# apache/paimon

Hardware: NVIDIA H100
Metric: merged rows/sec at 16 runs x 40M rows (higher is better)
Workload: dtype int64

## Files before the change

paimon_b200/csrc/device_utils.cuh:

```cuda
#pragma once

#include "pg_internal.h"

namespace pg {

__device__ __forceinline__ int warp_scan_incl(int v) {
    int lane = threadIdx.x & 31;
#pragma unroll
    for (int d = 1; d < 32; d <<= 1) {
        int n = __shfl_up_sync(0xffffffffu, v, d);
        if (lane >= d) v += n;
    }
    return v;
}

__device__ __forceinline__ int block_scan_excl(int v, int *ws, int *total) {
    int lane = threadIdx.x & 31, w = threadIdx.x >> 5, nw = blockDim.x >> 5;
    int incl = warp_scan_incl(v);
    if (lane == 31) ws[w] = incl;
    __syncthreads();
    if (w == 0) {
        int x = lane < nw ? ws[lane] : 0;
        int xi = warp_scan_incl(x);
        ws[lane] = xi - x;
// ... 120 lines not shown
    }
    if (fn == 4) {
        r = -(__int128)a;
    } else if (fn == 2) {
        r = dec_div_half_up((__int128)a * (__int128)b, dec_pow10(scale));
    } else {
        if (b == 0) {
            atomicCAS(err, KERR_NONE, a == 0 ? KERR_DEC_DIV_UNDEFINED : KERR_DEC_DIV_ZERO);
            return DecimalResult{0, false};
        }
        const uint64_t mb = b < 0 ? 0ull - ub : ub;
        uint64_t x = a < 0 ? 0ull - ua : ua, y = mb;
        while (x != 0) { const uint64_t t = y % x; y = x; x = t; }
        uint64_t den = mb / y;
        while (den % 2 == 0) den /= 2;
        while (den % 5 == 0) den /= 5;
        if (den != 1) {
            atomicCAS(err, KERR_NONE, KERR_DEC_NON_TERMINATING);
            return DecimalResult{0, false};
        }
        const __int128 n = (__int128)a * (__int128)dec_pow10(scale);
        r = dec_div_half_up(b < 0 ? -n : n, (unsigned __int128)mb);
    }
    const bool fits = dec_fits(r, precision);
    return DecimalResult{fits ? (uint64_t)(int64_t)r : 0, fits};
}

__device__ __forceinline__ uint64_t negate_fixed(int type, int width, uint64_t a) {
    if (type == PG_DOUBLE) return a ^ 0x8000000000000000ull;
    if (type == PG_FLOAT) return (uint32_t)a ^ 0x80000000u;
    return 0ull - (uint64_t)sext(a, width);
}

__device__ __forceinline__ int compare_fixed(int type, int width, uint64_t a, uint64_t b) {
    if (type == PG_DOUBLE)
        return java_double_compare(__longlong_as_double((long long)a), __longlong_as_double((long long)b));
    if (type == PG_FLOAT) return java_float_compare(__int_as_float((int)a), __int_as_float((int)b));
    int64_t x = sext(a, width), y = sext(b, width);
    return x < y ? -1 : x > y ? 1 : 0;
}

__device__ __forceinline__ int bytes_compare(const uint8_t *a, int la, const uint8_t *b, int lb) {
    int n = min(la, lb);
    for (int i = 0; i < n; i++) {
        int d = (int)a[i] - (int)b[i];
        if (d) return d;
    }
    return la - lb;
}


__device__ __forceinline__ uint32_t smem_u32(const void *p) { return (uint32_t)__cvta_generic_to_shared(p); }

__device__ __forceinline__ void mbar_init(uint64_t *bar, int count) {
    asm volatile("mbarrier.init.shared::cta.b64 [%0], %1;" ::"r"(smem_u32(bar)), "r"(count) : "memory");
}
__device__ __forceinline__ void mbar_fence_init() {
    asm volatile("fence.mbarrier_init.release.cluster;" ::: "memory");
    asm volatile("fence.proxy.async.shared::cta;" ::: "memory");
}
__device__ __forceinline__ void mbar_arrive_expect_tx(uint64_t *bar, uint32_t bytes) {
    asm volatile("mbarrier.arrive.expect_tx.shared::cta.b64 _, [%0], %1;" ::"r"(smem_u32(bar)), "r"(bytes)
                 : "memory");
}
__device__ __forceinline__ void mbar_wait(uint64_t *bar, uint32_t parity) {
    uint32_t ok;
    do {
        asm volatile(
            "{\n\t.reg .pred p;\n\t"
            "mbarrier.try_wait.parity.shared::cta.b64 p, [%1], %2;\n\t"
            "selp.u32 %0, 1, 0, p;\n\t}"
            : "=r"(ok)
            : "r"(smem_u32(bar)), "r"(parity)
            : "memory");
    } while (!ok);
}
__device__ __forceinline__ void bulk_g2s(void *dst_smem, const void *src_gmem, uint32_t bytes, uint64_t *bar) {
    asm volatile("cp.async.bulk.shared::cluster.global.mbarrier::complete_tx::bytes [%0], [%1], %2, [%3];" ::"r"(
                     smem_u32(dst_smem)),
                 "l"(src_gmem), "r"(bytes), "r"(smem_u32(bar))
                 : "memory");
}

}
```

paimon_b200/csrc/emit.cu:

```cuda
#include <stdio.h>

#include "device_utils.cuh"

namespace pg {

constexpr int kStages = 2;
constexpr int kEmitThreads = 512;
constexpr int kEmitWarps = kEmitThreads / 32;
#define kFlagAgg (1ull << 62)
#define kFlagPrefix (2ull << 62)
#define kValMask ((1ull << 62) - 1)

constexpr uint32_t kPmPosMask = 0x1FFF;
constexpr int kPmOpShift = 13;
constexpr uint32_t kPmHead = 0x8000;

struct EmitLayout {
    int rt;
    size_t stage_bytes;
    size_t total;
};
__host__ __device__ inline EmitLayout emit_layout(int k) {
    EmitLayout L;
    L.rt = kTileMax + 64 * k;
    L.stage_bytes = (((size_t)L.rt * 8 + (size_t)L.rt / 32 * 4) + 127) & ~(size_t)127;
    L.total = kStages * L.stage_bytes + (size_t)kTileMax * (2 + 2 + 1) + (PG_MAX_RUNS + 1) * 4 * 3 +
              PG_MAX_RUNS * 8 + kStages * PG_MAX_RUNS * 8 + kStages * 8 + 34 * 4 + 64;
    return L;
}

__device__ __forceinline__ bool staged_valid(const uint32_t *vw, int p) { return (vw[p >> 5] >> (p & 31)) & 1; }

template <int W> __device__ __forceinline__ uint64_t lds_fixed(const unsigned char *vals, int p);
template <> __device__ __forceinline__ uint64_t lds_fixed<1>(const unsigned char *v, int p) { return v[p]; }
template <> __device__ __forceinline__ uint64_t lds_fixed<2>(const unsigned char *v, int p) { return ((const uint16_t *)v)[p]; }
template <> __device__ __forceinline__ uint64_t lds_fixed<4>(const unsigned char *v, int p) { return ((const uint32_t *)v)[p]; }
template <> __device__ __forceinline__ uint64_t lds_fixed<8>(const unsigned char *v, int p) { return ((const uint64_t *)v)[p]; }
template <typename T> __device__ __forceinline__ T *as_global(T *p) { __builtin_assume(__isGlobal(p)); return p; }
template <int W> __device__ __forceinline__ void stg_fixed(void *d, int64_t row, uint64_t v);
template <> __device__ __forceinline__ void stg_fixed<1>(void *d, int64_t r, uint64_t v) { as_global((uint8_t *)d)[r] = (uint8_t)v; }
template <> __device__ __forceinline__ void stg_fixed<2>(void *d, int64_t r, uint64_t v) { as_global((uint16_t *)d)[r] = (uint16_t)v; }
template <> __device__ __forceinline__ void stg_fixed<4>(void *d, int64_t r, uint64_t v) { as_global((uint32_t *)d)[r] = (uint32_t)v; }
template <> __device__ __forceinline__ void stg_fixed<8>(void *d, int64_t r, uint64_t v) { as_global((uint64_t *)d)[r] = v; }

template <bool GAGG>
__device__ __forceinline__ int select_pos(const uint16_t *pm, const uint32_t *vw, int last) {
    int j = last;
    while (true) {
        uint32_t e = pm[j];
        uint32_t op = (e >> kPmOpShift) & 3;
        if (GAGG && op == OP_RETRACT) op = (e & kPmHead) ? OP_SET : OP_NOOP;
        if (op != OP_NOOP) {
            int pj = e & kPmPosMask;
            if (staged_valid(vw, pj)) return pj;
            if (op == OP_SET) return -1;
        }
        if (e & kPmHead) return -1;
        --j;
    }
}
template <bool GAGG>
__device__ __forceinline__ int select_member_idx(const uint16_t *pm, const uint32_t *vw, int last) {
    int j = last;
    while (true) {
        uint32_t e = pm[j];
        uint32_t op = (e >> kPmOpShift) & 3;
        if (GAGG && op == OP_RETRACT) op = (e & kPmHead) ? OP_SET : OP_NOOP;
        if (op != OP_NOOP) {
            if (staged_valid(vw, e & kPmPosMask)) return j;
            if (op == OP_SET) return -1;
        }
        if (e & kPmHead) return -1;
        --j;
    }
}

__device__ __forceinline__ int select_marked_idx(const uint16_t *pm, const uint32_t *gplan, uint32_t bit, int last) {
    int j = last;
    while (true) {
        if (gplan[j] & bit) return j;
        if (pm[j] & kPmHead) return -1;
        --j;
    }
}

__device__ __forceinline__ int group_first(const uint16_t *pm, int last) {
    int j = last;
    while (!(pm[j] & kPmHead)) --j;
    return j;
}

__device__ int fold_member_idx(const ColDesc &cd, const uint16_t *pm, const uint8_t *mrun, const uint32_t *vw,
                               const int32_t *offs, const uint8_t *const *cdata, int last, int32_t *err) {
    int acc = -1;
    bool initialized = false;
    for (int j = group_first(pm, last); j <= last; j++) {
        uint32_t e = pm[j];
        int op = (e >> kPmOpShift) & 3;
        if (op == OP_NOOP) continue;
        bool v = staged_valid(vw, e & kPmPosMask);
        int in = v ? j : -1;
        if (op == OP_SET) { acc = in; continue; }
        if (op == OP_RETRACT) {
            if (cd.retract == RT_IGNORE) continue;
            switch (cd.agg) {
                case PG_AGG_LAST_VALUE: acc = -1; break;
                case PG_AGG_LAST_NON_NULL_VALUE: if (v) acc = -1; break;
                case PG_AGG_PRIMARY_KEY: acc = in; break;
                default: atomicCAS(err, KERR_NONE, KERR_AGG_RETRACT); break;
            }
// ... 213 lines not shown
        if (active) {
            uint64_t val = 0;
            const int last = tv.glast[ob];
            if (cd.mode == CM_SELECT) {
                int pj = select_pos<GAGG>(tv.pm, vw, last);
                if (pj >= 0) { val = lds_fixed<W>(vals, pj); is_valid = true; }
            } else if (cd.mode == CM_GVAL || cd.mode == CM_GSEQ) {
                const uint32_t gbit = 1u << (cd.agg + (cd.mode == CM_GSEQ ? 16 : 0));
                const int j = select_marked_idx(tv.pm, ea.gplan + tv.in_base, gbit, last);
                if (j >= 0) {
                    const int pj = tv.pm[j] & kPmPosMask;
                    if (staged_valid(vw, pj)) { val = lds_fixed<W>(vals, pj); is_valid = true; }
                }
            } else if (GAGG && cd.mode == CM_GAGG) {
                fold_group_agg<false>(cd, tv.pm, ea.gagg + tv.in_base, vw, vals, last, &val, &is_valid, ea.err);
                if (!is_valid) val = 0;
            } else if (cd.mode == CM_KEY) {
                val = lds_fixed<W>(vals, tv.pm[last] & kPmPosMask); is_valid = true;
            } else if (cd.mode == CM_SEQ) {
                val = (uint64_t)ea.tmp_seq[result_index(tv, ob)]; is_valid = true;
            } else if (cd.mode == CM_KIND) {
                val = (uint8_t)ea.tmp_kind[result_index(tv, ob)]; is_valid = true;
            } else {
                fold_fixed<false>(cd, tv.pm, vw, vals, last, &val, &is_valid, ea.err);
                if (!is_valid) val = 0;
            }
            stg_fixed<W>(oc.data, tv.out_base + ob, val);
        }
        if (oc.validity != nullptr) put_validity_word(oc.validity, tv.out_base, wb, tv.n_out, is_valid);
    }
}

template <bool GAGG>
__device__ __forceinline__ void emit_decimal_column(const ColDesc &cd, const pg_out_column &oc, const TileView &tv,
                                                    const unsigned char *vals, const uint32_t *vw, const uint32_t *gagg,
                                                    int32_t *err) {
    const int tid = threadIdx.x, lane = tid & 31;
    for (int wb = (tid & ~31) - tv.o_shift; wb < tv.n_out; wb += kEmitThreads) {
        const int ob = wb + lane;
        bool is_valid = false;
        if (ob >= 0 && ob < tv.n_out) {
            uint64_t val = 0;
            const int last = tv.glast[ob];
            if (GAGG && cd.mode == CM_GAGG) fold_group_agg<true>(cd, tv.pm, gagg, vw, vals, last, &val, &is_valid, err);
            else fold_fixed<true>(cd, tv.pm, vw, vals, last, &val, &is_valid, err);
            stg_fixed<8>(oc.data, tv.out_base + ob, is_valid ? val : 0);
        }
        if (oc.validity != nullptr) put_validity_word(oc.validity, tv.out_base, wb, tv.n_out, is_valid);
    }
}

#ifdef PG_EMIT_TIMING
__device__ long long g_emit_ts[64 * 256];
#define TS(slot) do { if (tid == 0 && ts_on) g_emit_ts[(ts_tile) * 256 + (slot)] = clock64(); } while (0)
#else
#define TS(slot) do { } while (0)
#endif

struct PassEnt { ColDesc cd; pg_out_column oc; int32_t c, pad; };
constexpr int kPassCache = 64;

template <bool GAGG>
__global__ void __launch_bounds__(kEmitThreads, 2)
k_emit(EmitArgs ea) {
    extern __shared__ __align__(128) unsigned char smem[];
    __shared__ PassEnt s_pass[kPassCache];
    const int k = ea.k, tid = threadIdx.x, lane = tid & 31, warp = tid >> 5;
    const EmitLayout L = emit_layout(k);
    auto stage_vals = [&](int s) -> unsigned char * { return smem + (size_t)s * L.stage_bytes; };
    auto stage_vw = [&](int s) -> uint32_t * { return (uint32_t *)(smem + (size_t)s * L.stage_bytes + (size_t)L.rt * 8); };
    unsigned char *p = smem + kStages * L.stage_bytes;
    uint16_t *pm = (uint16_t *)p;              p += kTileMax * 2;
    uint16_t *glast = (uint16_t *)p;           p += kTileMax * 2;
    uint8_t *mrun = (uint8_t *)p;              p += kTileMax;
    int64_t *rstart = (int64_t *)p;            p += PG_MAX_RUNS * 8;
    const uint8_t **cdata = (const uint8_t **)p; p += kStages * PG_MAX_RUNS * 8;
    uint64_t *mbar = (uint64_t *)p;            p += kStages * 8;
    int64_t *s_i64 = (int64_t *)p;             p += 16;
    int *seg = (int *)p;                       p += (PG_MAX_RUNS + 1) * 4;
    int *seg_a = (int *)p;                     p += (PG_MAX_RUNS + 1) * 4;
    int *rr = (int *)p;                        p += (PG_MAX_RUNS + 1) * 4;
    int *ws = (int *)p;                        p += 34 * 4;
    int *s_i32 = (int *)p;                     p += 16;

    if (tid == 0) {
        s_i32[0] = atomicAdd(ea.tile_counter, 1);
        for (int s = 0; s < kStages; s++) mbar_init(&mbar[s], 1);
        mbar_fence_init();
    }
    __syncthreads();
    const int tile = s_i32[0];
    if (tid < ea.n_passes && tid < kPassCache) {
        const int c = ea.col_order[tid];
        s_pass[tid].c = c;
        s_pass[tid].cd = ea.cols[c];
        s_pass[tid].oc = ea.out_cols[c];
    }
#ifdef PG_EMIT_TIMING
    const bool ts_on = tile >= 2000 && tile < 2064;
    const int ts_tile = tile - 2000;
#endif
    TS(0);
    const int plan_a = 2 * tile, plan_end = min(plan_a + 2, ea.n_plan_tiles);
    if (warp == 0) {
        int64_t b0 = 0, bm = 0, b1 = 0;
        if (lane < k) {
            b0 = ea.bounds[(int64_t)plan_a * k + lane];
            bm = ea.bounds[(int64_t)(plan_a + 1) * k + lane];
            b1 = ea.bounds[(int64_t)plan_end * k + lane];
        }
        const int len = (int)(b1 - b0), len_a = (int)(bm - b0);
        const int rlen = lane < k ? (((int)(b0 & 31) + len + 1) + 31) & ~31 : 0;
        const int i_len = warp_scan_incl(len), i_a = warp_scan_incl(len_a), i_r = warp_scan_incl(rlen);
        if (lane < k) {
            rstart[lane] = b0;
            seg[lane] = i_len - len;
            seg_a[lane] = i_a - len_a;
            rr[lane] = i_r - rlen;
        }
        if (lane == 31) { seg[k] = i_len; seg_a[k] = i_a; rr[k] = i_r; }
    }
    __syncthreads();
    const int n = seg[k];
    const int n_vw = rr[k] >> 5;
    int64_t in_base = 0;
    for (int r = 0; r < k; r++) in_base += rstart[r];

    constexpr int VT = kTileMax / kEmitThreads;
    const int p0 = tid * VT, p1 = min(p0 + VT, n);
    int my = 0;
    uint32_t emit_bits = 0;
    uint16_t *spos = glast;
    uint8_t *srun = stage_vals(1);
    const int n_a = seg_a[k];
    for (int r = 0; r < k; r++) {
        const int len_a = seg_a[r + 1] - seg_a[r], len = seg[r + 1] - seg[r];
        const int p0r = rr[r] + (int)(rstart[r] & 31);
        const int sb0 = n_a + (seg[r] - seg_a[r]);
        for (int j = tid; j < len; j += kEmitThreads) {
            const int idx = j < len_a ? seg_a[r] + j : sb0 + (j - len_a);
            spos[idx] = (uint16_t)(p0r + j);
            srun[idx] = (uint8_t)r;
        }
    }
    __syncthreads();
    for (int i = p0; i < p1; i++) {
        uint16_t e = ea.plan[in_base + i];
        int slot = (e & kPlanSlotMask) + (i < n_a ? 0 : n_a);
        mrun[i] = srun[slot];
        uint32_t pos = spos[slot];
        uint32_t op = (e >> kPlanOpShift) & 3;
        pm[i] = (uint16_t)(pos | (op << kPmOpShift) | ((e & kPlanHead) ? kPmHead : 0));
        if ((e & kPlanHead) && (e & kPlanEmit)) { my++; emit_bits |= 1u << (i - p0); }
    }
    int n_out = 0;
    int o = block_scan_excl(my, ws, &n_out);
    for (int i = p0; i < p1; i++) {
        if (emit_bits & (1u << (i - p0))) {
            int e = i + 1;
            while (e < n && !(pm[e] & kPmHead)) e++;
            glast[o++] = (uint16_t)(e - 1);
        }
    }
    int vw_run = -1;
    int64_t vw_gword = 0;
    if (tid < n_vw) {
        int r = 0;
        while (r + 1 < k && (rr[r + 1] >> 5) <= tid) r++;
        vw_run = r;
        vw_gword = (rstart[r] >> 5) + (tid - (rr[r] >> 5));
        if (vw_gword > ((ea.run_rows[r] - 1) >> 5)) vw_run = -1;
    }
    __syncthreads();

    TileView tv;
    tv.pm = pm;
    tv.glast = glast;
    tv.n_out = n_out;
    tv.out_base = ea.row_base[plan_a];
    tv.o_shift = (int)(tv.out_base & 31);
    tv.in_base = in_base;
    tv.n_out_a = ea.tile_rows[plan_a];
    tv.seq_shift = n_a - tv.n_out_a;
    const int ncols = ea.n_passes;
    uint32_t phase = 0;

    auto col_staged = [&](const ColDesc &cd) { return cd.mode != CM_SEQ && cd.mode != CM_KIND; };
    auto pass_col = [&](int ci) -> int { return ci < kPassCache ? s_pass[ci].c : ea.col_order[ci]; };
    auto pass_desc = [&](int ci, int c) -> ColDesc { return ci < kPassCache ? s_pass[ci].cd : ea.cols[c]; };

    auto issue = [&](int c, const ColDesc &cd, int s) {
        if (!col_staged(cd)) return;
        asm volatile("fence.proxy.async.shared::cta;" ::: "memory");
        uint32_t bytes = 0;
        const unsigned char *src = nullptr;
        unsigned char *dst = nullptr;
        if (lane < k) {
            const int r = lane;
            const int len = seg[r + 1] - seg[r];
            const int64_t row0 = rstart[r] & ~(int64_t)31;
            const int head = (int)(rstart[r] & 31);
            if (cd.width > 0) {
                if (len > 0) {
                    bytes = (uint32_t)(((head + len) * cd.width + 15) & ~15);
                    src = (const unsigned char *)ea.ptrs.data[(int64_t)c * k + r] + row0 * cd.width;
                    dst = stage_vals(s) + (size_t)rr[r] * cd.width;
                }
            } else {
                if (len > 0) {
                    bytes = (uint32_t)(((head + len + 1) * 4 + 15) & ~15);
                    src = (const unsigned char *)(ea.ptrs.offsets[(int64_t)c * k + r] + row0);
                    dst = stage_vals(s) + (size_t)rr[r] * 4;
                }
                cdata[s * PG_MAX_RUNS + r] = (const uint8_t *)ea.ptrs.data[(int64_t)c * k + r];
            }
        }
        uint32_t total = bytes;
#pragma unroll
        for (int d = 16; d > 0; d >>= 1) total += __shfl_xor_sync(0xffffffffu, total, d);
        if (lane == 0) mbar_arrive_expect_tx(&mbar[s], total);
        __syncwarp();
        if (bytes) bulk_g2s(dst, src, bytes, &mbar[s]);
    };
    auto load_vw = [&](int c) -> uint32_t {
        if (vw_run < 0) return 0xffffffffu;
        const uint32_t *vp = ea.ptrs.validity[(int64_t)c * k + vw_run];
        return vp ? vp[vw_gword] : 0xffffffffu;
    };

    if (warp == 0 && ncols > 0) issue(pass_col(0), pass_desc(0, pass_col(0)), 0);
    if (tid < n_vw && ncols > 0) stage_vw(0)[tid] = load_vw(pass_col(0));
    __syncthreads();

    TS(1);
    for (int ci = 0; ci < ncols; ci++) {
        const int s = ci & 1;
        const int c = pass_col(ci);
        const int cn = ci + 1 < ncols ? pass_col(ci + 1) : -1;
        const ColDesc cd = pass_desc(ci, c);
        const pg_out_column oc = ci < kPassCache ? s_pass[ci].oc : ea.out_cols[c];
        if (warp == 0 && cn >= 0) issue(cn, pass_desc(ci + 1, cn), s ^ 1);
        uint32_t next_vw = (cn >= 0 && tid < n_vw) ? load_vw(cn) : 0;
        if (col_staged(cd)) {
            mbar_wait(&mbar[s], (phase >> s) & 1);
            phase ^= 1u << s;
        }
        const unsigned char *vals = stage_vals(s);
        const uint32_t *vw = stage_vw(s);

        if (cd.decimal) emit_decimal_column<GAGG>(cd, oc, tv, vals, vw, GAGG ? ea.gagg + tv.in_base : nullptr, ea.err);
        else if (cd.width == 8) emit_fixed_column<8, GAGG>(ea, cd, oc, tv, vals, vw);
        else if (cd.width == 4) emit_fixed_column<4, GAGG>(ea, cd, oc, tv, vals, vw);
        else if (cd.width == 1) emit_fixed_column<1, GAGG>(ea, cd, oc, tv, vals, vw);
        else if (cd.width == 2) emit_fixed_column<2, GAGG>(ea, cd, oc, tv, vals, vw);
        else {
            const int32_t *offs = (const int32_t *)vals;
            uint16_t *vsrc = (uint16_t *)(vals + (size_t)L.rt * 4);
            int *wpre = (int *)(vsrc + kTileMax);
            const uint8_t **wsrc = (const uint8_t **)(wpre + ((kEmitWarps * 33 + 1) & ~1));
            int *wend = (int *)(wsrc + kEmitWarps * 32);
            int64_t *wtot = (int64_t *)(wend + kEmitWarps * 32);
            static_assert(kTileMax * 2 + ((kEmitWarps * 33 + 1) & ~1) * 4 + kEmitWarps * 32 * (8 + 4) + kEmitWarps * 8 <=
                              (kTileMax + 64) * 4, "var-len scratch fits the upper half of a stage at k = 1");
            const uint8_t *const *cd_data = cdata + s * PG_MAX_RUNS;
            const int span = tv.o_shift + n_out;
            const int RW = (((span + kEmitWarps - 1) / kEmitWarps) + 31) & ~31;
            const int wbeg = -tv.o_shift + warp * RW;
            int64_t my_bytes = 0;
            for (int ob0 = wbeg; ob0 < wbeg + RW && ob0 < n_out; ob0 += 32) {
                const int ob = ob0 + lane;
                if (ob >= 0 && ob < n_out) {
                    const int last = glast[ob];
                    int src;
                    if (cd.mode == CM_KEY) src = last;
                    else if (cd.mode == CM_FOLD) src = fold_member_idx(cd, pm, mrun, vw, offs, cd_data, last, ea.err);
                    else if (cd.mode == CM_GVAL || cd.mode == CM_GSEQ) {
                        src = select_marked_idx(pm, ea.gplan + in_base,
                                                1u << (cd.agg + (cd.mode == CM_GSEQ ? 16 : 0)), last);
                        if (src >= 0 && !staged_valid(vw, pm[src] & kPmPosMask)) src = -1;
                    } else src = select_member_idx<GAGG>(pm, vw, last);
                    vsrc[ob] = src < 0 ? (uint16_t)0xFFFF : (uint16_t)src;
                    if (src >= 0) { int ps = pm[src] & kPmPosMask; my_bytes += offs[ps + 1] - offs[ps]; }
                }
            }
#pragma unroll
            for (int d = 16; d > 0; d >>= 1) my_bytes += __shfl_xor_sync(0xffffffffu, my_bytes, d);
            if (lane == 0) wtot[warp] = my_bytes;
            __syncthreads();
            if (ci < 60) TS(8 + 4 * ci + 0);
            uint64_t *state = ea.vl_state + (int64_t)cd.varlen_index * ea.n_tiles;
            if (warp == 0) {
                const int64_t x = lane < kEmitWarps ? wtot[lane] : 0;
                int64_t xi = x;
#pragma unroll
                for (int d = 1; d < kEmitWarps; d <<= 1) {
                    const int64_t y = __shfl_up_sync(0xffffffffu, xi, d);
                    if (lane >= d) xi += y;
                }
                const uint64_t tile_bytes = (uint64_t)__shfl_sync(0xffffffffu, xi, kEmitWarps - 1);
                if (lane < kEmitWarps) ws[lane] = (int)(xi - x);
                uint64_t excl = 0;
                if (lane == 0 && tile > 0) {
                    __threadfence();
                    atomicExch((unsigned long long *)&state[tile], kFlagAgg | (uint64_t)tile_bytes);
                }
                constexpr int kLook = 8;
                int t = tile - 1;
                while (t >= 0) {
                    uint64_t sv[kLook];
#pragma unroll
                    for (int q = 0; q < kLook; q++) {
                        const int idx = t - (lane * kLook + q);
                        sv[q] = idx >= 0 ? *((volatile uint64_t *)&state[idx]) : kFlagPrefix;
                    }
                    int lp = 32 * kLook;
#pragma unroll
                    for (int q = kLook - 1; q >= 0; q--) if ((unsigned)(sv[q] >> 62) == 2) lp = lane * kLook + q;
                    int first = lp;
#pragma unroll
                    for (int d = 16; d > 0; d >>= 1) first = min(first, __shfl_xor_sync(0xffffffffu, first, d));
                    bool inval = false;
                    uint64_t contrib = 0;
#pragma unroll
                    for (int q = 0; q < kLook; q++) {
                        if (lane * kLook + q <= first) {
                            if ((unsigned)(sv[q] >> 62) == 0) inval = true;
                            contrib += sv[q] & kValMask;
                        }
                    }
                    if (__any_sync(0xffffffffu, inval)) continue;
#pragma unroll
                    for (int d = 16; d > 0; d >>= 1) contrib += __shfl_xor_sync(0xffffffffu, contrib, d);
                    excl += contrib;
                    if (first < 32 * kLook) break;
                    t -= 32 * kLook;
                }
                if (lane == 0) {
                    __threadfence();
                    const uint64_t tot = excl + tile_bytes;
                    atomicExch((unsigned long long *)&state[tile], kFlagPrefix | tot);
                    const bool fits = tot <= 0x7fffffffull;
                    if (!fits) atomicCAS(ea.err, KERR_NONE, KERR_OFFSET_OVERFLOW);
                    s_i64[0] = fits ? (int64_t)excl : -1;
                    if (tile == ea.n_tiles - 1) {
                        ea.totals[1 + cd.varlen_index] = (int64_t)tot;
                        if (fits) oc.offsets[ea.totals[0]] = (int32_t)tot;
                    }
                }
            }
            __syncthreads();
            if (ci < 60) TS(8 + 4 * ci + 1);
            const int64_t byte_base = s_i64[0];
            uint8_t *dbase = (uint8_t *)oc.data + (byte_base < 0 ? 0 : byte_base);
            int carry = ws[warp];
            int *my_pre = wpre + warp * 33;
            int *my_end = wend + warp * 32;
            const uint8_t **my_src = wsrc + warp * 32;
            const int ob_end = byte_base < 0 ? wbeg : min(wbeg + RW, n_out);
            for (int ob0 = wbeg; ob0 < ob_end; ob0 += 32) {
                const int ob = ob0 + lane;
                const bool active = ob >= 0 && ob < n_out;
                int len = 0;
                const uint8_t *sp = nullptr;
                bool has = false;
                if (active) {
                    int src = vsrc[ob];
                    if (src != 0xFFFF) {
                        int ps = pm[src] & kPmPosMask;
                        int st = offs[ps];
                        len = offs[ps + 1] - st;
                        sp = cd_data[mrun[src]] + st;
                        has = true;
                    }
                }
                const int incl = warp_scan_incl(len);
                const int off = carry + incl - len;
                carry += __shfl_sync(0xffffffffu, incl, 31);
                if (active) oc.offsets[tv.out_base + ob] = (int32_t)(byte_base + off);
                if (oc.validity != nullptr) put_validity_word(oc.validity, tv.out_base, ob0, n_out, has);
                const unsigned pay = __ballot_sync(0xffffffffu, len > 0);
                const int n_pay = __popc(pay);
                if (len > 0) {
                    const int ci = __popc(pay & ((1u << lane) - 1));
                    my_pre[ci] = off;
                    my_end[ci] = off + len;
                    my_src[ci] = sp;
                }
                __syncwarp();
                for (int rg = 0; rg < n_pay; rg += 8) {
                    const int ra = rg + (lane >> 3), rb = ra + 4;
                    int a0 = 0, a1 = 0, b0 = 0, b1 = 0;
                    const uint8_t *pa = nullptr, *pb = nullptr;
                    if (ra < n_pay) { a0 = my_pre[ra]; a1 = my_end[ra]; pa = my_src[ra] - a0; }
                    if (rb < n_pay) { b0 = my_pre[rb]; b1 = my_end[rb]; pb = my_src[rb] - b0; }
                    const int64_t ia = (int64_t)a0 + (lane & 7), ib = (int64_t)b0 + (lane & 7);
                    uint8_t xa0 = 0, xa1 = 0, xa2 = 0, xb0 = 0, xb1 = 0, xb2 = 0;
                    if (ia < a1) xa0 = pa[ia];
                    if (ia + 8 < a1) xa1 = pa[ia + 8];
                    if (ia + 16 < a1) xa2 = pa[ia + 16];
                    if (ib < b1) xb0 = pb[ib];
                    if (ib + 8 < b1) xb1 = pb[ib + 8];
                    if (ib + 16 < b1) xb2 = pb[ib + 16];
                    if (ia < a1) dbase[ia] = xa0;
                    if (ia + 8 < a1) dbase[ia + 8] = xa1;
                    if (ia + 16 < a1) dbase[ia + 16] = xa2;
                    if (ib < b1) dbase[ib] = xb0;
                    if (ib + 8 < b1) dbase[ib + 8] = xb1;
                    if (ib + 16 < b1) dbase[ib + 16] = xb2;
                    for (int64_t b = ia + 24; b < a1; b += 8) dbase[b] = pa[b];
                    for (int64_t b = ib + 24; b < b1; b += 8) dbase[b] = pb[b];
                }
                __syncwarp();
            }
        }
        if (cn >= 0 && tid < n_vw) stage_vw(s ^ 1)[tid] = next_vw;
        __syncthreads();
        if (ci < 60) TS(8 + 4 * ci + 3);
    }
}

#ifdef PG_EMIT_TIMING
void emit_timing_dump() {
    static long long h[64 * 256];
    cudaDeviceSynchronize();
    cudaMemcpyFromSymbol(h, g_emit_ts, sizeof(h));
    double acc[256] = {0};
    int cntv[256] = {0};
    for (int t = 0; t < 64; t++)
        for (int sl = 1; sl < 256; sl++) {
            if (h[t * 256 + sl] == 0) continue;
            int pv = sl - 1;
            while (pv > 0 && h[t * 256 + pv] == 0) pv--;
            if (h[t * 256 + pv] == 0) continue;
            acc[sl] += (double)(h[t * 256 + sl] - h[t * 256 + pv]);
            cntv[sl]++;
        }
    fprintf(stderr, "[emit timing] cycles since previous slot (avg over tiles):");
    for (int sl = 1; sl < 256; sl++) if (cntv[sl]) fprintf(stderr, " %d:%.0f", sl, acc[sl] / cntv[sl]);
    fprintf(stderr, "\n");
    static long long z[64 * 256];
    cudaMemcpyToSymbol(g_emit_ts, z, sizeof(z));
}
#endif

static bool g_emit_attr = false;
void launch_emit(const EmitArgs &ea) {
    EmitLayout L = emit_layout(ea.k);
    if (!g_emit_attr) {
        cudaFuncSetAttribute(k_emit<false>, cudaFuncAttributeMaxDynamicSharedMemorySize, 200 * 1024);
        cudaFuncSetAttribute(k_emit<true>, cudaFuncAttributeMaxDynamicSharedMemorySize, 200 * 1024);
        g_emit_attr = true;
    }
    if (ea.gagg) k_emit<true><<<ea.n_tiles, kEmitThreads, L.total, ea.stream>>>(ea);
    else k_emit<false><<<ea.n_tiles, kEmitThreads, L.total, ea.stream>>>(ea);
#ifdef PG_EMIT_TIMING
    emit_timing_dump();
#endif
}

}
```

paimon_b200/csrc/parquet_decode.cu:

```cuda
#include <algorithm>
#include <cstring>
#include <memory>
#include <stdexcept>

#include "device_utils.cuh"
#include "parquet_meta.h"
#include "inflate_device.cuh"
#include "lz4_device.cuh"
#include "snappy_device.cuh"
#include "scan_kernels.cuh"
#include "zstd_device.cuh"

namespace pg {

enum : int { ENC_PLAIN = 0, ENC_DICT = 1, ENC_DELTA_BP = 2, ENC_RLE_BOOL = 3 };

struct PqChunk {
    const uint8_t *base;
    int64_t avail;
    int64_t num_values;
    int64_t row0;
    int32_t col, run, file, codec;
    int32_t max_def, phys, phys_width;
    int32_t cast;
// ... 597 lines not shown
            const int64_t x = i < last ? pages[i].payload_bytes : 0;
            int64_t incl = x;
#pragma unroll
            for (int d = 1; d < 32; d <<= 1) {
                const int64_t y = __shfl_up_sync(0xffffffffu, incl, d);
                if (lane >= d) incl += y;
            }
            if (i < last) {
                pages[i].payload_base = carry + incl - x;
                pages[i].vs_base = pr.vs_rows_base + pages[i].row0 + i + pr.idx;
                pages[i].is_last = i == last - 1;
            }
            carry += __shfl_sync(0xffffffffu, incl, 31);
        }
    }
    if (lane == 0) {
        totals[w] = carry;
        if (carry > 0x7fffffffLL) pq_err(err, KERR_OFFSET_OVERFLOW);
    }
}

constexpr int kWalkWindow = 2048;
constexpr int kWalkWarps = 8;

template <typename Emit>
__device__ int64_t pq_walk_stream(const uint8_t *stream, int64_t stream_len, int count, uint8_t *win, uint32_t *w_off,
                                  int32_t *w_len, Emit emit) {
    const int lane = threadIdx.x & 31;
    int done = 0;
    int64_t pos = 0;
    while (done < count) {
        if (pos + 4 > stream_len) return -1;
        const uint8_t *p = stream + pos;
        const uint8_t *base = (const uint8_t *)((uintptr_t)p & ~(uintptr_t)15);
        const int skip = (int)(p - base);
        const int avail = (int)min((int64_t)(stream + stream_len - base), (int64_t)(kWalkWindow + 16));
        for (int o = lane * 16; o < avail; o += 32 * 16) *(uint4 *)(win + o) = *(const uint4 *)(base + o);
        __syncwarp();
        int nfound = 0, q = skip;
        bool corrupt = false;
        if (lane == 0) {
            while (done + nfound < count && q + 4 <= avail && nfound < 256) {
                const int32_t len = (int32_t)((uint32_t)win[q] | ((uint32_t)win[q + 1] << 8) | ((uint32_t)win[q + 2] << 16) |
                                              ((uint32_t)win[q + 3] << 24));
                if (len < 0) { corrupt = true; break; }
                w_off[nfound] = (uint32_t)q;
                w_len[nfound] = len;
                nfound++;
                if ((int64_t)q + 4 + len > 0x7fffffff) { corrupt = true; break; }
                q += 4 + len;
            }
        }
        nfound = __shfl_sync(0xffffffffu, nfound, 0);
        q = __shfl_sync(0xffffffffu, q, 0);
        corrupt = __shfl_sync(0xffffffffu, (int)corrupt, 0);
        __syncwarp();
        const int64_t base_off = (int64_t)(base - stream);
        for (int i = lane; i < nfound; i += 32) emit(done + i, base_off + w_off[i], w_len[i]);
        __syncwarp();
        if (corrupt || nfound == 0) return -1;
        done += nfound;
        pos = base_off + q;
        if (pos > stream_len) return -1;
    }
    return pos;
}

__global__ void __launch_bounds__(kWalkWarps * 32)
k_pq_walk_dicts(const PqPage *dicts, int n_dicts, const PqChunk *chunks, int32_t *dict_off, int32_t *dict_len, int32_t *err) {
    __shared__ __align__(16) uint8_t s_win[kWalkWarps][kWalkWindow + 32];
    __shared__ uint32_t s_off[kWalkWarps][256];
    __shared__ int32_t s_len[kWalkWarps][256];
    const int w = threadIdx.x >> 5, lane = threadIdx.x & 31;
    const int t = blockIdx.x * kWalkWarps + w;
    if (t >= n_dicts) return;
    const PqPage dj = dicts[t];
    if (chunks[dj.chunk].phys != pq::T_BYTE_ARRAY) return;
    int32_t *doff = dict_off + dj.entry_base, *dlen = dict_len + dj.entry_base;
    const int64_t endq = pq_walk_stream(dj.body, dj.body_len, dj.num_values, s_win[w], s_off[w], s_len[w],
                                        [&](int j, int64_t q, int32_t len) { doff[j] = (int32_t)(q + 4); dlen[j] = len; });
    if (lane == 0 && endq < 0) pq_err(err, KERR_BAD_PAGE);
}

__device__ __forceinline__ void cp_async16(void *smem_dst, const void *gsrc) {
    asm volatile("cp.async.cg.shared.global [%0], [%1], 16;" ::"r"((uint32_t)__cvta_generic_to_shared(smem_dst)), "l"(gsrc) : "memory");
}
__device__ __forceinline__ void cp_async4(void *smem_dst, const void *gsrc) {
    asm volatile("cp.async.ca.shared.global [%0], [%1], 4;" ::"r"((uint32_t)__cvta_generic_to_shared(smem_dst)), "l"(gsrc) : "memory");
}
__device__ __forceinline__ void cp_async_commit() { asm volatile("cp.async.commit_group;" ::: "memory"); }
template <int N> __device__ __forceinline__ void cp_async_wait() { asm volatile("cp.async.wait_group %0;" ::"n"(N) : "memory"); }
constexpr int kWvWarps = 1;
constexpr int kWvChunk = 128, kWvRing = 4, kWvLead = 1, kWvCap = 32;
constexpr int kWvRow = kWvChunk * kWvRing;
static_assert(kWvCap == 32, "one lane's values of a step leave as one warp store");
static_assert((kWvRow & (kWvRow - 1)) == 0 && kWvChunk == 8 * 16 && kWvRow / 16 >= 16, "power-of-two ring, 8 units per chunk");

#ifdef PG_WALK_TIMING
constexpr int kWtSlots = 256;
__device__ long long g_walk_ts[kWtSlots][8];
#define WT_DECL long long wt_t = 0, wt_acc[3] = {0, 0, 0}, wt_steps = 0, wt_g0 = 0; \
    const int wt_slot = (blockIdx.x % 4 == 0 && blockIdx.x < 4 * kWtSlots) ? (int)(blockIdx.x / 4) : -1; \
    if (wt_slot >= 0) { asm volatile("mov.u64 %0, %%globaltimer;" : "=l"(wt_g0)); wt_t = clock64(); }
#define WT_MARK(k) do { if (wt_slot >= 0) { const long long wt_n = clock64(); wt_acc[k] += wt_n - wt_t; wt_t = wt_n; \
    if ((k) == 2) wt_steps++; } } while (0)
#define WT_END(vals) do { if (wt_slot >= 0) { long long wt_v = (vals); \
    for (int d = 16; d > 0; d >>= 1) wt_v += __shfl_xor_sync(0xffffffffu, wt_v, d); \
    if ((threadIdx.x & 31) == 0 && wt_v > 0) { long long g1; asm volatile("mov.u64 %0, %%globaltimer;" : "=l"(g1)); \
        unsigned smid; asm("mov.u32 %0, %%smid;" : "=r"(smid)); long long *o = g_walk_ts[wt_slot]; \
        o[0] = wt_acc[0]; o[1] = wt_acc[1]; o[2] = wt_acc[2]; o[3] = wt_steps; o[4] = wt_v; o[5] = wt_g0; o[6] = g1; \
        o[7] = smid; } } } while (0)
#else
#define WT_DECL
#define WT_MARK(k) do {} while (0)
#define WT_END(vals) do {} while (0)
#endif

__global__ void __launch_bounds__(kWvWarps * 32)
k_pq_walk_values(PqPage *pages, int n_pages, const PqChunk *chunks, int32_t *vstart, int32_t *err) {
    __shared__ __align__(16) uint8_t s_ring[kWvWarps][32][kWvRow];
    __shared__ const uint8_t *s_req_src[kWvWarps][32 * kWvRing];
    __shared__ uint32_t s_req_dst[kWvWarps][32 * kWvRing];
    __shared__ int32_t s_vs[kWvWarps][32][kWvCap + 1];
    const int lane = threadIdx.x & 31, warp = threadIdx.x >> 5;
    const int t = blockIdx.x * (kWvWarps * 32) + threadIdx.x;
    WT_DECL
    bool done = true;
    PqPage pg;
    pg.nnz = 0;
    if (t < n_pages) {
        pg = pages[t];
        done = pg.bad || pg.enc != ENC_PLAIN || chunks[pg.chunk].phys != pq::T_BYTE_ARRAY;
    }
    const bool mine = !done;
    const uint8_t *stream = mine ? pg.body + pg.values_off : nullptr;
    const int32_t slen = mine ? pg.body_len - pg.values_off : 0;
    const int nnz = mine ? pg.nnz : 0;
    const uint8_t *a0 = (const uint8_t *)((uintptr_t)stream & ~(uintptr_t)15);
    const uint32_t off0 = (uint32_t)(stream - a0);
    uint32_t p = off0, pend = off0 + (uint32_t)max(slen, 0);
    uint32_t bias = mine ? (uint32_t)pg.payload_base - off0 : 0;
    int32_t *vs = mine ? vstart + pg.vs_base : nullptr;
    int j = 0;
    bool bad = slen < 0;
    if (nnz == 0 || bad) done = true;
    const int n_chunks = done ? 0 : (int)((pend + kWvChunk - 1) / kWvChunk);
    int next = 0;
    int hist[kWvLead + 1];
#pragma unroll
    for (int i = 0; i <= kWvLead; i++) hist[i] = 0;
    uint8_t (*rows)[kWvRow] = s_ring[warp];
    const uint8_t *row = rows[lane];
    const int sw = lane & 15;
    while (true) {
        cp_async_wait<kWvLead>();
        __syncwarp();
        WT_MARK(1);
        const uint32_t lim = (uint32_t)hist[0] * kWvChunk;
        const int j0 = j;
        if (!done) {
            for (int c = 0; c < kWvCap; c++) {
                if (p + 4 > pend) { bad = true; break; }
                if (p + 4 > lim) break;
                const uint32_t wi = (p >> 2) & (kWvRow / 4 - 1), wj = (wi + 1) & (kWvRow / 4 - 1);
                const uint32_t lo = *(const uint32_t *)(row + ((((wi >> 2) ^ sw) << 4) | ((wi & 3) << 2)));
                const uint32_t hi = *(const uint32_t *)(row + ((((wj >> 2) ^ sw) << 4) | ((wj & 3) << 2)));
                const uint32_t len = __funnelshift_r(lo, hi, (p & 3) * 8);
                if (len > pend - p - 4) { bad = true; break; }
                s_vs[warp][lane][c] = (int32_t)(p + bias);
                bias -= 4;
                p += 4 + len;
                if (++j == nnz) break;
            }
            if (bad || j == nnz) done = true;
// ... 986 lines not shown
```

Before: 896.4 million.

## Prefetch per-run column pointers and validity words asynchronously with cp.async

The emit kernel now stages each column's per-run data, offset and validity pointers into shared memory with cp.async two passes ahead, instead of reading them from global memory right before issuing the bulk copy. Validity words for the next column are also fetched with cp.async straight into the stage buffer, replacing a register load followed by a later store. The aim is to take dependent global pointer loads off the critical path of each column pass. The cost is extra shared memory, more commit/wait groups and a full cp.async wait before the first issue. The cp.async helpers move into a shared header, and a profiling script plus retimed TS markers are added.

```diff
diff --git a/paimon_b200/csrc/device_utils.cuh b/paimon_b200/csrc/device_utils.cuh
--- a/paimon_b200/csrc/device_utils.cuh
+++ b/paimon_b200/csrc/device_utils.cuh
@@ -226,4 +226,16 @@
                  : "memory");
 }
 
-}
+__device__ __forceinline__ void cp_async16(void *smem_dst, const void *gsrc) {
+    asm volatile("cp.async.cg.shared.global [%0], [%1], 16;" ::"r"((uint32_t)__cvta_generic_to_shared(smem_dst)), "l"(gsrc) : "memory");
+}
+__device__ __forceinline__ void cp_async8(void *smem_dst, const void *gsrc) {
+    asm volatile("cp.async.ca.shared.global [%0], [%1], 8;" ::"r"((uint32_t)__cvta_generic_to_shared(smem_dst)), "l"(gsrc) : "memory");
+}
+__device__ __forceinline__ void cp_async4(void *smem_dst, const void *gsrc) {
+    asm volatile("cp.async.ca.shared.global [%0], [%1], 4;" ::"r"((uint32_t)__cvta_generic_to_shared(smem_dst)), "l"(gsrc) : "memory");
+}
+__device__ __forceinline__ void cp_async_commit() { asm volatile("cp.async.commit_group;" ::: "memory"); }
+template <int N> __device__ __forceinline__ void cp_async_wait() { asm volatile("cp.async.wait_group %0;" ::"n"(N) : "memory"); }
+
+}
diff --git a/paimon_b200/csrc/emit.cu b/paimon_b200/csrc/emit.cu
--- a/paimon_b200/csrc/emit.cu
+++ b/paimon_b200/csrc/emit.cu
@@ -25,7 +25,7 @@
     L.rt = kTileMax + 64 * k;
     L.stage_bytes = (((size_t)L.rt * 8 + (size_t)L.rt / 32 * 4) + 127) & ~(size_t)127;
     L.total = kStages * L.stage_bytes + (size_t)kTileMax * (2 + 2 + 1) + (PG_MAX_RUNS + 1) * 4 * 3 +
-              PG_MAX_RUNS * 8 + kStages * PG_MAX_RUNS * 8 + kStages * 8 + 34 * 4 + 64;
+              PG_MAX_RUNS * 8 + kStages * PG_MAX_RUNS * 8 + kStages * 2 * (size_t)k * 8 + kStages * 8 + 34 * 4 + 40;
     return L;
 }
 
@@ -405,6 +405,8 @@
     int *rr = (int *)p;                        p += (PG_MAX_RUNS + 1) * 4;
     int *ws = (int *)p;                        p += 34 * 4;
     int *s_i32 = (int *)p;                     p += 16;
+    p = (unsigned char *)(((uintptr_t)p + 7) & ~(uintptr_t)7);
+    const void **s_ptr = (const void **)p;     p += kStages * 2 * k * 8;
 
     if (tid == 0) {
         s_i32[0] = atomicAdd(ea.tile_counter, 1);
@@ -485,14 +487,12 @@
             glast[o++] = (uint16_t)(e - 1);
         }
     }
-    int vw_run = -1;
-    int64_t vw_gword = 0;
+    int vw_key = -1;
     if (tid < n_vw) {
         int r = 0;
         while (r + 1 < k && (rr[r + 1] >> 5) <= tid) r++;
-        vw_run = r;
-        vw_gword = (rstart[r] >> 5) + (tid - (rr[r] >> 5));
-        if (vw_gword > ((ea.run_rows[r] - 1) >> 5)) vw_run = -1;
+        const int w = tid - (rr[r] >> 5);
+        if ((rstart[r] >> 5) + w <= ((ea.run_rows[r] - 1) >> 5)) vw_key = w << 5 | r;
     }
     __syncthreads();
 
@@ -511,6 +511,19 @@
     auto col_staged = [&](const ColDesc &cd) { return cd.mode != CM_SEQ && cd.mode != CM_KIND; };
     auto pass_col = [&](int ci) -> int { return ci < kPassCache ? s_pass[ci].c : ea.col_order[ci]; };
     auto pass_desc = [&](int ci, int c) -> ColDesc { return ci < kPassCache ? s_pass[ci].cd : ea.cols[c]; };
+
+    auto run_ptr = [&](int s, int t, int r) -> const void * { return s_ptr[(s * 2 + t) * k + r]; };
+    auto fetch_ptrs = [&](int ci, int s) {
+        if (tid < 2 * k) {
+            const int c = pass_col(ci);
+            const int t = tid >= k, r = tid - t * k;
+            const void *const *tab = t ? (const void *const *)ea.ptrs.validity
+                                   : (ci < kPassCache ? s_pass[ci].cd.width : ea.cols[c].width) > 0
+                                         ? ea.ptrs.data : (const void *const *)ea.ptrs.offsets;
+            cp_async8(&s_ptr[(s * 2 + t) * k + r], tab + (int64_t)c * k + r);
+            cp_async_commit();
+        }
+    };
 
     auto issue = [&](int c, const ColDesc &cd, int s) {
         if (!col_staged(cd)) return;
@@ -526,16 +539,17 @@
             if (cd.width > 0) {
                 if (len > 0) {
                     bytes = (uint32_t)(((head + len) * cd.width + 15) & ~15);
-                    src = (const unsigned char *)ea.ptrs.data[(int64_t)c * k + r] + row0 * cd.width;
+                    src = (const unsigned char *)run_ptr(s, 0, r) + row0 * cd.width;
                     dst = stage_vals(s) + (size_t)rr[r] * cd.width;
                 }
             } else {
                 if (len > 0) {
                     bytes = (uint32_t)(((head + len + 1) * 4 + 15) & ~15);
-                    src = (const unsigned char *)(ea.ptrs.offsets[(int64_t)c * k + r] + row0);
+                    src = (const unsigned char *)((const int32_t *)run_ptr(s, 0, r) + row0);
                     dst = stage_vals(s) + (size_t)rr[r] * 4;
                 }
-                cdata[s * PG_MAX_RUNS + r] = (const uint8_t *)ea.ptrs.data[(int64_t)c * k + r];
+                cp_async8(&cdata[s * PG_MAX_RUNS + r], &ea.ptrs.data[(int64_t)c * k + r]);
+                cp_async_commit();
             }
         }
         uint32_t total = bytes;
@@ -545,14 +559,25 @@
         __syncwarp();
         if (bytes) bulk_g2s(dst, src, bytes, &mbar[s]);
     };
-    auto load_vw = [&](int c) -> uint32_t {
-        if (vw_run < 0) return 0xffffffffu;
-        const uint32_t *vp = ea.ptrs.validity[(int64_t)c * k + vw_run];
-        return vp ? vp[vw_gword] : 0xffffffffu;
+    auto load_vw = [&](int s, uint32_t *dst) {
+        const uint32_t *vp = nullptr;
+        int r = 0;
+        if (vw_key >= 0) {
+            r = vw_key & 31;
+            vp = (const uint32_t *)run_ptr(s, 1, r);
+        }
+        if (vp) cp_async4(dst, vp + (rstart[r] >> 5) + (vw_key >> 5));
+        else *dst = 0xffffffffu;
+        cp_async_commit();
     };
 
+    if (ncols > 0) fetch_ptrs(0, 0);
+    if (ncols > 1) fetch_ptrs(1, 1);
+    cp_async_wait<0>();
+    __syncthreads();
     if (warp == 0 && ncols > 0) issue(pass_col(0), pass_desc(0, pass_col(0)), 0);
-    if (tid < n_vw && ncols > 0) stage_vw(0)[tid] = load_vw(pass_col(0));
+    if (tid < n_vw && ncols > 0) load_vw(0, stage_vw(0) + tid);
+    cp_async_wait<0>();
     __syncthreads();
 
     TS(1);
@@ -563,11 +588,13 @@
         const ColDesc cd = pass_desc(ci, c);
         const pg_out_column oc = ci < kPassCache ? s_pass[ci].oc : ea.out_cols[c];
         if (warp == 0 && cn >= 0) issue(cn, pass_desc(ci + 1, cn), s ^ 1);
-        uint32_t next_vw = (cn >= 0 && tid < n_vw) ? load_vw(cn) : 0;
+        if (cn >= 0 && tid < n_vw) load_vw(s ^ 1, stage_vw(s ^ 1) + tid);
+        if (ci + 2 < ncols) fetch_ptrs(ci + 2, s);
         if (col_staged(cd)) {
             mbar_wait(&mbar[s], (phase >> s) & 1);
             phase ^= 1u << s;
         }
+        if (ci < 60) TS(8 + 4 * ci + 0);
         const unsigned char *vals = stage_vals(s);
         const uint32_t *vw = stage_vw(s);
 
@@ -610,7 +637,7 @@
             for (int d = 16; d > 0; d >>= 1) my_bytes += __shfl_xor_sync(0xffffffffu, my_bytes, d);
             if (lane == 0) wtot[warp] = my_bytes;
             __syncthreads();
-            if (ci < 60) TS(8 + 4 * ci + 0);
+            if (ci < 60) TS(8 + 4 * ci + 1);
             uint64_t *state = ea.vl_state + (int64_t)cd.varlen_index * ea.n_tiles;
             if (warp == 0) {
                 const int64_t x = lane < kEmitWarps ? wtot[lane] : 0;
@@ -672,7 +699,7 @@
                 }
             }
             __syncthreads();
-            if (ci < 60) TS(8 + 4 * ci + 1);
+            if (ci < 60) TS(8 + 4 * ci + 2);
             const int64_t byte_base = s_i64[0];
             uint8_t *dbase = (uint8_t *)oc.data + (byte_base < 0 ? 0 : byte_base);
             int carry = ws[warp];
@@ -736,7 +763,7 @@
                 __syncwarp();
             }
         }
-        if (cn >= 0 && tid < n_vw) stage_vw(s ^ 1)[tid] = next_vw;
+        cp_async_wait<0>();
         __syncthreads();
         if (ci < 60) TS(8 + 4 * ci + 3);
     }
diff --git a/paimon_b200/csrc/parquet_decode.cu b/paimon_b200/csrc/parquet_decode.cu
--- a/paimon_b200/csrc/parquet_decode.cu
+++ b/paimon_b200/csrc/parquet_decode.cu
@@ -703,14 +703,6 @@
     if (lane == 0 && endq < 0) pq_err(err, KERR_BAD_PAGE);
 }
 
-__device__ __forceinline__ void cp_async16(void *smem_dst, const void *gsrc) {
-    asm volatile("cp.async.cg.shared.global [%0], [%1], 16;" ::"r"((uint32_t)__cvta_generic_to_shared(smem_dst)), "l"(gsrc) : "memory");
-}
-__device__ __forceinline__ void cp_async4(void *smem_dst, const void *gsrc) {
-    asm volatile("cp.async.ca.shared.global [%0], [%1], 4;" ::"r"((uint32_t)__cvta_generic_to_shared(smem_dst)), "l"(gsrc) : "memory");
-}
-__device__ __forceinline__ void cp_async_commit() { asm volatile("cp.async.commit_group;" ::: "memory"); }
-template <int N> __device__ __forceinline__ void cp_async_wait() { asm volatile("cp.async.wait_group %0;" ::"n"(N) : "memory"); }
 constexpr int kWvWarps = 1;
 constexpr int kWvChunk = 128, kWvRing = 4, kWvLead = 1, kWvCap = 32;
 constexpr int kWvRow = kWvChunk * kWvRing;
diff --git a/profiles/emit_passes.py b/profiles/emit_passes.py
--- /dev/null
+++ b/profiles/emit_passes.py
@@ -0,0 +1,135 @@
+import argparse
+import json
+import os
+import re
+import subprocess
+import sys
+import tempfile
+
+ROOT = os.path.dirname(os.path.dirname(os.path.abspath(__file__)))
+PHASES = ("wait", "pass 1", "look-back", "pass 2")
+
+
+def build_timing_lib(build_dir):
+    build_dir = os.path.abspath(build_dir)
+    lib = os.path.join(build_dir, "libpaimon_gpu.so")
+    subprocess.check_call(["make", "-C", ROOT, "-j8", f"OBJDIR={build_dir}", "EXTRA_DEFS=-DPG_EMIT_TIMING",
+                           f"LIB={lib}", lib])
+    return lib
+
+
+def parse_dump(text):
+    dumps = []
+    for line in text.splitlines():
+        if line.startswith("[emit timing]"):
+            dumps.append({int(a): float(b) for a, b in re.findall(r" (\d+):([0-9.]+)", line)})
+    return dumps
+
+
+def split_passes(dump):
+    varlen, fixed = [], []
+    for ci in range(60):
+        b = 8 + 4 * ci
+        if b + 3 not in dump:
+            continue
+        if b + 1 in dump:
+            varlen.append({"wait": dump.get(b, 0.0), "pass 1": dump[b + 1], "look-back": dump.get(b + 2, 0.0),
+                           "pass 2": dump[b + 3]})
+        else:
+            fixed.append({"wait": dump.get(b, 0.0), "pass 2": dump[b + 3]})
+    return varlen, fixed
+
+
+def worker(args):
+    sys.path.insert(0, ROOT)
+    os.environ.setdefault("PG_RUN_CACHE_BYTES", str(64 << 30))
+    import torch
+    import bench
+    from paimon_b200 import _native as N
+    from paimon_b200.sort_merge_reader import SortMergeReader
+    dev = torch.device("cuda", 0)
+    torch.cuda.set_device(dev)
+    N.init(0)
+    schema = bench.make_schema("c3")
+    spec = bench.make_spec("c3", schema)
+    readers, _, _, _ = bench.device_runs("c3", schema, args.rows, dev, seed=100)
+    rd = SortMergeReader.create_sort_merge_reader(readers, None, None, spec, device=0)
+    log = tempfile.TemporaryFile(mode="w+")
+    saved = os.dup(2)
+    sampler = bench.ClockSampler(0)
+    try:
+        rd.execute()
+        sys.stderr.flush()
+        os.dup2(log.fileno(), 2)
+        sampler.start()
+        for _ in range(args.merges):
+            rd.execute()
+        torch.cuda.synchronize()
+        clocks = sampler.stop()
+        n_tiles = rd.stats().n_tiles
+        sys.stderr.flush()
+    finally:
+        os.dup2(saved, 2)
+        os.close(saved)
+        rd.close()
+    log.seek(0)
+    dumps = parse_dump(log.read())
+    if len(dumps) != args.merges:
+        raise SystemExit(f"expected {args.merges} emit timing dumps, got {len(dumps)}: is this a -DPG_EMIT_TIMING build?")
+    q = subprocess.run(["nvidia-smi", "--id=0", "--query-gpu=name,power.limit,clocks.max.sm", "--format=csv,noheader"],
+                       capture_output=True, text=True).stdout.strip()
+    res = {"gpu": q, "sm_mhz_median": clocks.get("sm_mhz"), "clock_reasons": clocks.get("reasons"),
+           "n_tiles": n_tiles}
+    for kind, idx in (("varlen", 0), ("fixed", 1)):
+        per_merge = [split_passes(d)[idx] for d in dumps]
+        n = len(per_merge[0])
+        res[kind] = {"passes_per_tile": n,
+                     "mean_cycles": {ph: sum(p[ph] for m in per_merge for p in m if ph in p) / max(1, n * len(dumps))
+                                     for ph in PHASES if any(ph in p for m in per_merge for p in m)}}
+    json.dump(res, sys.stdout)
+
+
+def main():
+    ap = argparse.ArgumentParser()
+    ap.add_argument("--lib", action="append", default=[], metavar="NAME=PATH",
+                    help="a -DPG_EMIT_TIMING build of libpaimon_gpu.so (repeatable)")
+    ap.add_argument("--build-dir", default=os.path.join(ROOT, "build", "emit_timing"))
+    ap.add_argument("--merges", type=int, default=3)
+    ap.add_argument("--rows", type=int, default=40_000_000)
+    ap.add_argument("--out", default=None, help="also write emit_passes.json here")
+    ap.add_argument("--worker", action="store_true", help=argparse.SUPPRESS)
+    args = ap.parse_args()
+    if args.worker:
+        return worker(args)
+    libs = [tuple(x.split("=", 1)) for x in args.lib] or [("timing", build_timing_lib(args.build_dir))]
+    results = {}
+    for name, path in libs:
+        env = dict(os.environ, PAIMON_GPU_LIB=os.path.abspath(path))
+        out = subprocess.run([sys.executable, os.path.abspath(__file__), "--worker", "--merges", str(args.merges),
+                              "--rows", str(args.rows)], env=env, capture_output=True, text=True, cwd=ROOT)
+        if out.returncode != 0:
+            sys.stderr.write(out.stderr[-4000:])
+            raise SystemExit(f"{name}: worker failed ({out.returncode})")
+        results[name] = json.loads(out.stdout.strip().splitlines()[-1])
+    first = next(iter(results.values()))
+    print(f"GPU: {first['gpu']} (name, power limit, max SM clock); SM clock median during the merges: "
+          f"{first['sm_mhz_median']} MHz {first['clock_reasons']}")
+    print(f"k_emit, C3 at {args.rows} rows: mean cycles per (tile, pass) of thread 0 over 64 tiles x {args.merges} merges")
+    print("| build | passes | n/tile | " + " | ".join(PHASES) + " | sum | us/pass |")
+    print("|---|---|---|" + "---|" * (len(PHASES) + 2))
+    for name, r in results.items():
+        mhz = r["sm_mhz_median"] or 0
+        for kind in ("varlen", "fixed"):
+            m = r[kind]["mean_cycles"]
+            tot = sum(m.values())
+            cells = " | ".join(f"{m[ph]:.0f}" if ph in m else "-" for ph in PHASES)
+            us = f"{tot / mhz:.1f}" if mhz else "n/a"
+            print(f"| {name} | {kind} | {r[kind]['passes_per_tile']} | {cells} | {tot:.0f} | {us} |")
+    if args.out:
+        os.makedirs(args.out, exist_ok=True)
+        with open(os.path.join(args.out, "emit_passes.json"), "w") as f:
+            json.dump(results, f, indent=1)
+
+
+if __name__ == "__main__":
+    main()
```

Result: no change. 904.8 million (median of 6 runs) (+0.9%).
